# RDLLab/posggym-baselines

Measured on AMD Instinct MI355X. Metric: MCTS simulations/sec on Driving-v1 (POMCP exact search), higher is better.
Workload: dtype f64

## Files before the change

### posggym-baselines_amd/csrc/driving.h

```cpp
#pragma once
#include <stdint.h>

#include "philox.h"

namespace pb {

enum : int { NORTH = 0, EAST = 1, SOUTH = 2, WEST = 3 };
enum : int { REVERSE = 0, STOPPED = 1, FORWARD_SLOW = 2, FORWARD_FAST = 3 };
enum : int { DO_NOTHING = 0, ACCELERATE = 1, DECELERATE = 2, TURN_RIGHT = 3, TURN_LEFT = 4 };
enum : int { CELL_VEHICLE = 0, CELL_WALL = 1, CELL_EMPTY = 2, CELL_DEST = 3 };

struct DrvGrid {
  uint8_t wall[256];
  uint8_t dist[8][256];
  uint8_t loc_x[8], loc_y[8], loc_dir[8];
  int32_t width, height, num_locs;
  int32_t obs_front, obs_back, obs_side;
  int32_t pad[2];
};

struct Veh {
  int x, y, dir, speed, dest, reached, crashed, mind, initd;
};

// ... 140 lines not shown
  v.crashed = 0;
  v.mind = g.dist[dest][(v.y << 4) | v.x];
  v.initd = v.mind;
  return pack_veh(v);
}

PB_HD int kth_bit(uint32_t mask, uint32_t k) {
  for (int i = 0; i < 8; ++i) {
    if (mask & (1u << i)) {
      if (k == 0) return i;
      --k;
    }
  }
  return -1;
}

PB_HD int popc8(uint32_t m) {
  int n = 0;
  for (int i = 0; i < 8; ++i) n += (m >> i) & 1;
  return n;
}

template <class G, class Draw>
PB_HD void drv_sample_initial_state2(const G& g, Draw draw, uint32_t* s0, uint32_t* s1) {
  const uint32_t all = (1u << g.num_locs) - 1u;
  uint32_t starts = 0, dests = 0;
  uint32_t out[2];
  for (int i = 0; i < 2; ++i) {
    const uint32_t av = all & ~starts;
    const int s = kth_bit(av, draw((uint32_t)popc8(av)));
    starts |= 1u << s;
    const uint32_t avd = all & ~dests & ~(1u << s);
    const int d = kth_bit(avd, draw((uint32_t)popc8(avd)));
    dests |= 1u << d;
    out[i] = make_vehicle(g, s, d);
  }
  *s0 = out[0];
  *s1 = out[1];
}

template <class G>
PB_HD int loc_index(const G& g, int x, int y) {
  for (int k = 0; k < g.num_locs; ++k)
    if (g.loc_x[k] == x && g.loc_y[k] == y) return k;
  return -1;
}

}

namespace pb {

struct DrvModel {
  DrvGrid g;
  uint16_t win_wall[1024];
  uint16_t nbr2[1024];
  double prog[3 * 128];
};

template <class G>
PB_HD void build_model_tables(const G& g, DrvModel* m) {
  const int ncells = (g.obs_front + g.obs_back + 1) * (2 * g.obs_side + 1);
  for (int cell = 0; cell < 256; ++cell) {
    const int x = cell & 15, y = cell >> 4;
    for (int d = 0; d < 4; ++d) {
      const int nx = x + dir_dx(d), ny = y + dir_dy(d);
      int n1 = 0xFF, n2 = 0xFF;
      if (grid_free(g, nx, ny)) {
        n1 = (ny << 4) | nx;
        const int mx = nx + dir_dx(d), my = ny + dir_dy(d);
        if (grid_free(g, mx, my)) n2 = (my << 4) | mx;
      }
      m->nbr2[cell * 4 + d] = (uint16_t)(n1 | (n2 << 8));
      uint32_t w = 0;
      const int W = 2 * g.obs_side + 1;
      const int r = (d + 1) & 3;
      for (int c = 0; c < ncells; ++c) {
        const int fwd = g.obs_front - c / W;
        const int side = c % W - g.obs_side;
        const int cx = x + fwd * dir_dx(d) + side * dir_dx(r);
        const int cy = y + fwd * dir_dy(d) + side * dir_dy(r);
        if (!grid_free(g, cx, cy)) w |= 1u << c;
      }
      m->win_wall[cell * 4 + d] = (uint16_t)w;
    }
  }
  for (int k = 0; k < 3; ++k)
    for (int i = 0; i < 128; ++i)
      m->prog[k * 128 + i] = i == 0 ? 0.0 : (0.5 * (double)k) / (double)i;
}

PB_HD int window_index(const DrvGrid& g, int x, int y, int d, int tx, int ty) {
  const int rx = tx - x, ry = ty - y;
  const int r = (d + 1) & 3;
  const int fwd = rx * dir_dx(d) + ry * dir_dy(d);
  const int side = rx * dir_dx(r) + ry * dir_dy(r);
  if (fwd < -g.obs_back || fwd > g.obs_front || side < -g.obs_side || side > g.obs_side) return -1;
  return (g.obs_front - fwd) * (2 * g.obs_side + 1) + (side + g.obs_side);
}

PB_HD uint32_t spread_bits16(uint32_t x) {
  x &= 0xFFFFu;
  x = (x | (x << 8)) & 0x00FF00FFu;
  x = (x | (x << 4)) & 0x0F0F0F0Fu;
  x = (x | (x << 2)) & 0x33333333u;
  x = (x | (x << 1)) & 0x55555555u;
  return x;
}

PB_HD uint64_t obs_key_fast(const DrvModel& m, uint32_t self, uint32_t other) {
  const DrvGrid& g = m.g;
  const int ncells = (g.obs_front + g.obs_back + 1) * (2 * g.obs_side + 1);
  const uint32_t full = (1u << ncells) - 1u;
  const int x = self & 15, y = (self >> 4) & 15, d = (self >> 8) & 3;
  const uint32_t wall = m.win_wall[(((y << 4) | x) << 2) | d];
  uint32_t cells = spread_bits16(wall) | (spread_bits16(~wall & full) << 1);
  const int dest = (self >> 12) & 7;
  const int cd = window_index(g, x, y, d, g.loc_x[dest], g.loc_y[dest]);
  if (cd >= 0 && !((wall >> cd) & 1u)) cells |= 3u << (2 * cd);
  const int cv = window_index(g, x, y, d, (int)(other & 15), (int)((other >> 4) & 15));
  if (cv >= 0 && !((wall >> cv) & 1u)) cells &= ~(3u << (2 * cv));
  return (uint64_t)cells | obs_tail(g, self);
}

struct MovePlan {
  uint32_t self;
  int d, speed, cells;
  uint32_t path;
  bool done;
};

PB_HD MovePlan plan_move(const DrvModel& m, uint32_t self, int action) {
  MovePlan p;
  p.self = self;
  p.done = veh_done(self);
  int d = (self >> 8) & 3, speed = (self >> 10) & 3;
  if (action == TURN_RIGHT) d = (d + 1) & 3;
  else if (action == TURN_LEFT) d = (d + 3) & 3;
  else if (action == ACCELERATE) speed = speed + 1 < FORWARD_FAST ? speed + 1 : FORWARD_FAST;
  else if (action == DECELERATE) speed = speed - 1 > REVERSE ? speed - 1 : REVERSE;
  const int move = speed != REVERSE ? d : ((d + 2) & 3);
  p.d = d;
  p.speed = speed;
  p.cells = speed > STOPPED ? speed - STOPPED : STOPPED - speed;
  p.path = m.nbr2[((self & 0xFF) << 2) | (uint32_t)move];
  return p;
}

PB_HD int resolve_move(const MovePlan& p, int ocell, int* speed, bool* hit) {
  int cell = (int)(p.self & 0xFF);
  *speed = p.speed;
  *hit = false;
  if (p.cells >= 1) {
    const int c1 = (int)(p.path & 0xFF);
    if (c1 == 0xFF) {
      *speed = STOPPED;
    } else if (c1 == ocell) {
      *hit = true;
      *speed = STOPPED;
    } else {
      cell = c1;
      if (p.cells >= 2) {
        const int c2 = (int)(p.path >> 8);
        if (c2 == 0xFF) {
          *speed = STOPPED;
        } else if (c2 == ocell) {
          *hit = true;
          *speed = STOPPED;
        } else {
          cell = c2;
        }
      }
    }
  }
  return cell;
}

PB_HD uint32_t finish_move(const DrvModel& m, const MovePlan& p, int cell, int speed, bool hit) {
  const uint32_t self = p.self;
  const int dest = (self >> 12) & 7;
  const int dist = m.g.dist[dest][cell];
  const int mind0 = (self >> 17) & 127;
  const int mind = mind0 < dist ? mind0 : dist;
  return (self & 0x7F007000u) | (uint32_t)cell | ((uint32_t)p.d << 8) | ((uint32_t)speed << 10) |
         ((uint32_t)(dist == 0) << 15) | ((uint32_t)hit << 16) | ((uint32_t)mind << 17);
}

PB_HD void drv_step2_fast(const DrvModel& m, uint32_t s0, uint32_t s1, int a0, int a1, uint32_t j,
                          uint32_t* o0, uint32_t* o1) {
  const MovePlan p0 = plan_move(m, s0, a0);
  const MovePlan p1 = plan_move(m, s1, a1);
  const bool first1 = j == 0;
  const MovePlan& pf = first1 ? p1 : p0;
  const MovePlan& ps = first1 ? p0 : p1;
  uint32_t vf = pf.self, vs = ps.self;
  int cf = (int)(vf & 0xFF), cs = (int)(vs & 0xFF);
  int spf = 0, sps = 0;
  bool hf = false, hs = false, sec_crashed = false, fst_crashed = false;
  bool movedf = false, moveds = false;
  if (!pf.done) {
    cf = resolve_move(pf, cs, &spf, &hf);
    movedf = true;
    if (hf && !ps.done) sec_crashed = true;
  }
  if (!ps.done && !sec_crashed) {
    cs = resolve_move(ps, cf, &sps, &hs);
    moveds = true;
    if (hs) fst_crashed = true;
  }
  if (movedf) vf = finish_move(m, pf, cf, spf, hf);
  if (moveds) vs = finish_move(m, ps, cs, sps, hs);
  if (sec_crashed) vs |= 1u << 16;
  if (fst_crashed && !veh_done(vf)) vf |= 1u << 16;
  *o0 = first1 ? vs : vf;
  *o1 = first1 ? vf : vs;
}

PB_HD double drv_reward_fast(const DrvModel& m, uint32_t prev, uint32_t next) {
  if (veh_done(prev)) return 0.0;
  const double base = ((next >> 16) & 1) ? -1.0 : (((next >> 15) & 1) ? 0.5 : 0.0);
  const int progress = (int)((prev >> 17) & 127) - (int)((next >> 17) & 127);
  return base + m.prog[progress * 128 + (int)((prev >> 24) & 127)];
}

}
```

### posggym-baselines_amd/csrc/driving_vec.h

```cpp
#pragma once
#if defined(__HIPCC__)
#include <hip/hip_runtime.h>
#endif
#include <stdint.h>

#include "driving.h"

namespace pb {

PB_HD uint32_t vary(uint32_t x) {
#if defined(__HIP_DEVICE_COMPILE__)
  uint32_t r;
  asm("v_mov_b32 %0, %1" : "=v"(r) : "v"(x));
  return r;
#else
  return x;
#endif
}

struct VPlan {
  uint32_t self, path;
  uint32_t d, speed, cells, done;
};

// ... 21 lines not shown
struct VMove {
  uint32_t cell, speed, hit;
};

PB_HD VMove vresolve(const VPlan& p, uint32_t ocell) {
  const uint32_t c1 = p.path & 0xFFu, c2 = p.path >> 8;
  const uint32_t start = p.self & 0xFFu;
  const bool s1 = p.cells >= 1u;
  const bool w1 = c1 == 0xFFu, h1 = !w1 & (c1 == ocell);
  const bool a1 = s1 & !w1 & !h1;
  const bool s2 = (p.cells >= 2u) & a1;
  const bool w2 = c2 == 0xFFu, h2 = !w2 & (c2 == ocell);
  const bool a2 = s2 & !w2 & !h2;
  VMove r;
  r.cell = a2 ? c2 : (a1 ? c1 : start);
  r.hit = ((s1 & h1) | (s2 & h2)) ? 1u : 0u;
  r.speed = ((s1 & (w1 | h1)) | (s2 & (w2 | h2))) ? (uint32_t)STOPPED : p.speed;
  return r;
}

PB_HD uint32_t vfinish(const VPlan& p, const VMove& mv, uint32_t dist) {
  const uint32_t mind0 = (p.self >> 17) & 127u;
  const uint32_t mind = mind0 < dist ? mind0 : dist;
  return (p.self & 0x7F007000u) | mv.cell | (p.d << 8) | (mv.speed << 10) |
         ((dist == 0u ? 1u : 0u) << 15) | (mv.hit << 16) | (mind << 17);
}

PB_HD void drv_step2_vec(const DrvModel& m, uint32_t s0, uint32_t s1, uint32_t a0, uint32_t a1,
                         uint32_t j, uint32_t* o0, uint32_t* o1) {
  const bool first1 = j == 0u;
  const VPlan pf = vplan(m, first1 ? s1 : s0, first1 ? a1 : a0);
  const VPlan ps = vplan(m, first1 ? s0 : s1, first1 ? a0 : a1);
  const VMove mf = vresolve(pf, ps.self & 0xFFu);
  const bool movef = pf.done == 0u;
  const bool sec_crash = movef & (mf.hit != 0u) & (ps.done == 0u);
  const uint32_t cellf = movef ? mf.cell : (pf.self & 0xFFu);
  const VMove ms = vresolve(ps, cellf);
  const bool moves = (ps.done == 0u) & !sec_crash;
  const uint32_t cells = moves ? ms.cell : (ps.self & 0xFFu);
  const uint32_t distf = m.g.dist[(pf.self >> 12) & 7u][cellf];
  const uint32_t dists = m.g.dist[(ps.self >> 12) & 7u][cells];
  const uint32_t kf = movef ? ~0u : 0u, ks = moves ? ~0u : 0u;
  uint32_t vf = (vfinish(pf, mf, distf) & kf) | (pf.self & ~kf);
  uint32_t vs = (vfinish(ps, ms, dists) & ks) | (ps.self & ~ks);
  vs |= sec_crash ? (1u << 16) : 0u;
  const bool fst_crash = moves & (ms.hit != 0u) & (((vf >> 15) & 3u) == 0u);
  vf |= fst_crash ? (1u << 16) : 0u;
  *o0 = first1 ? vs : vf;
  *o1 = first1 ? vf : vs;
}

PB_HD double drv_reward_vec(const DrvModel& m, uint32_t prev, uint32_t next) {
  const uint32_t initd = (prev >> 24) & 127u;
  const double p1 = m.prog[128u + initd], p2 = m.prog[256u + initd];
  const bool done0 = ((prev >> 15) & 3u) != 0u;
  const double base = ((next >> 16) & 1u) ? -1.0 : (((next >> 15) & 1u) ? 0.5 : 0.0);
  const uint32_t progress = ((prev >> 17) & 127u) - ((next >> 17) & 127u);
  const double r = base + (progress == 1u ? p1 : (progress == 2u ? p2 : 0.0));
  return done0 ? 0.0 : r;
}

PB_HD int vwindow_index(const DrvGrid& g, int x, int y, int fx, int fy, int rx,
                                             int ry, int tx, int ty) {
  const int dx = tx - x, dy = ty - y;
  const int fwd = dx * fx + dy * fy;
  const int side = dx * rx + dy * ry;
  const bool in = fwd >= -g.obs_back && fwd <= g.obs_front && side >= -g.obs_side &&
                  side <= g.obs_side;
  return in ? (g.obs_front - fwd) * (2 * g.obs_side + 1) + (side + g.obs_side) : -1;
}

PB_HD uint64_t obs_key_vec(const DrvModel& m, uint32_t self, uint32_t other) {
  const DrvGrid& g = m.g;
  const int ncells = (g.obs_front + g.obs_back + 1) * (2 * g.obs_side + 1);
  const uint32_t full = (1u << ncells) - 1u;
  const int x = (int)(self & 15u), y = (int)((self >> 4) & 15u), d = (int)((self >> 8) & 3u);
  const uint32_t wall = m.win_wall[(self & 0xFFu) << 2 | (uint32_t)d];
  uint32_t cells = spread_bits16(wall) | (spread_bits16(~wall & full) << 1);
  const int fx = d == EAST ? 1 : (d == WEST ? -1 : 0);
  const int fy = d == SOUTH ? 1 : (d == NORTH ? -1 : 0);
  const int rx = -fy, ry = fx;
  const uint32_t dest = (self >> 12) & 7u;
  const int dxl = g.loc_x[dest], dyl = g.loc_y[dest];
  const int cd = vwindow_index(g, x, y, fx, fy, rx, ry, dxl, dyl);
  const uint32_t dmask = (cd >= 0 && !((wall >> (cd & 31)) & 1u)) ? (3u << (2 * (cd & 15))) : 0u;
  cells |= dmask;
  const int cv = vwindow_index(g, x, y, fx, fy, rx, ry, (int)(other & 15u), (int)((other >> 4) & 15u));
  const uint32_t vmask = (cv >= 0 && !((wall >> (cv & 31)) & 1u)) ? (3u << (2 * (cv & 15))) : 0u;
  cells &= ~vmask;
  const uint64_t tail = ((uint64_t)((self >> 10) & 3u) << 30) | ((uint64_t)x << 32) |
                        ((uint64_t)y << 36) | ((uint64_t)dxl << 40) | ((uint64_t)dyl << 44) |
                        ((uint64_t)((self >> 15) & 1u) << 48) | ((uint64_t)((self >> 16) & 1u) << 49);
  return (uint64_t)cells | tail;
}

}
```

### posggym-baselines_amd/csrc/pomcp_search.hip

```cpp
#pragma clang fp contract(off)

namespace pb {

constexpr int kMaxA = 5;
constexpr int kTPB = 256;
constexpr int kTPBSmall = 64;
#ifndef POMCP_ROOT_SLOTS_LDS
#define POMCP_ROOT_SLOTS_LDS 1
#endif
#ifndef POMCP_WAVES_PER_EU
#define POMCP_WAVES_PER_EU 1
#endif
constexpr bool kRootSlotsInLds = POMCP_ROOT_SLOTS_LDS != 0;
constexpr int kRootParts = kMaxA * (kRootSlotsInLds ? 1 + kSlots : 1);
__host__ __device__ constexpr int rc_stats(int a) { return a; }
__host__ __device__ constexpr int rc_slot(int a, int k) { return kMaxA + a * kSlots + k; }

constexpr int kRegPath = 3;
#ifndef PB_BQ_LEVELS
#define PB_BQ_LEVELS 3
#endif
constexpr int kBq = PB_BQ_LEVELS;
static_assert(kBq >= 1 && kBq <= kRegPath, "only register-path levels are queued (level() passes ql = -1 below)");
constexpr int kPre = 2 + kMaxA;
// ... 48 lines not shown
#endif
  const int wave = bx * (TPB / kWave) + (int)(threadIdx.x >> 6);
  const int tree = wave * kWave + lane;
  const bool valid = tree < p.B;
  const int tt = valid ? tree : 0;
  constexpr int A = NA;
  constexpr int L = blk_lines(NA, TM);
  char* const an = reinterpret_cast<char*>(p.an + tree_base_lines(tt, p.Nb, L));
  const int64_t blk_bytes = blk_stride_lines(L) * 128;
  const WaveLog wl(p.plog, p.Np, wave, TM);
  __shared__ __attribute__((aligned(16))) char tm_lds[TM != 0 ? sizeof(TmTables) : 16];
  if constexpr (TM != 0) {
    const uint32_t* src = reinterpret_cast<const uint32_t*>(p.tmt);
    uint32_t* dst = reinterpret_cast<uint32_t*>(tm_lds);
    for (int i = (int)threadIdx.x; i < (int)(sizeof(TmTables) / 4); i += TPB) dst[i] = src[i];
    __syncthreads();
  }
  const TmTables* const tmt = reinterpret_cast<const TmTables*>(tm_lds);
  uint32_t pid = 0;
  int epol = 0;
  const int islots = p.islots;
  const uint32_t slot_mask = (1u << islots) - 1u;
  const uint32_t wpos0 = p.wlog[wave];
  bool app = false;
  LogRec rec = {0u, 0u, 0u};
  __shared__ uint32_t wcnt[TPB / kWave];
  if (lane == 0) wcnt[threadIdx.x >> 6] = wpos0;
  __builtin_amdgcn_wave_barrier();
  auto append = [&]() {
    if (app) {
#ifndef POMCP_ABLATE_LOG
      const uint32_t at = atomicAdd(&wcnt[threadIdx.x >> 6], 1u);
      wl.store(at, rec);
      if constexpr (TM != 0) wl.aux[at] = pid;
#endif
      app = false;
    }
  };
  OvfSlot* const ovf = p.ovf + (int64_t)tt * p.H;
  PathEntry* const path = reinterpret_cast<PathEntry*>(p.path) + (int64_t)tt * kMaxPath;
  const TreeHdr* const h = p.hdr + tt;
  const int bdir = h->belief_sel ? -1 : 1;
  const uint4* const rbel = p.belief + (int64_t)tt * p.Nr + (h->belief_sel ? p.Nr - 1 : 0);
  int root_blk = h->root_blk, root_visits = h->root_visits;
  int n_blocks = h->n_blocks, n_log = h->n_log, n_nodes = h->n_nodes;
  const int bsize = h->belief_size, epoch = h->epoch, root_abs = h->root_abs;
  int err = h->error;
  double mm_min = h->mm_min, mm_max = h->mm_max;
  const uint64_t seed = uni64(h->seed);
  const uint32_t tkey = h->tree_key;
  uint32_t c_bel = h->ctr[0], c_sel = h->ctr[1], c_mod = h->ctr[2], c_a0 = h->ctr[3],
           c_a1 = h->ctr[4];
  const int log0 = n_log, blocks0 = n_blocks, nodes0 = n_nodes;
  int c_rollout = 0, c_probes = 0, c_cut = 0, c_exact = 0;
#ifdef POMCP_PHASE_TIMING
  uint64_t pt[16];
  for (int i = 0; i < 16; ++i) pt[i] = 0;
  uint64_t pt_last = __builtin_amdgcn_s_memtime();
#endif

  auto d_belief = [&](uint32_t n) { return uniform_int(philox_word(seed, tkey, S_BELIEF, c_bel++), n); };
  auto d_select = [&](uint32_t n) { return uniform_int(philox_word(seed, tkey, S_SELECT, c_sel++), n); };
  auto d_act_word = [&](int agent) {
    const bool a0 = agent == 0;
    const uint32_t j = a0 ? c_a0 : c_a1;
    c_a0 += a0 ? 1u : 0u;
    c_a1 += a0 ? 0u : 1u;
    return philox_word(seed, tkey, (uint32_t)S_ACT_BASE + (a0 ? 0u : 1u), j);
  };
  __shared__ uint32_t rw[2][4][TPB];
  uint32_t m_base = 0u, o_base = 0u;
  uint32_t w_bel = 0u;
  int pend_b = 0;
  uint32_t nm0 = 0u, nm1 = 0u, nm2 = 0u, nm3 = 0u, no0 = 0u, no1 = 0u, no2 = 0u, no3 = 0u;
  uint32_t nm_base = 0xFFFFFFFFu, no_base = 0xFFFFFFFFu;
  auto spec_blocks = [&]() {
    const uint32_t cm = m_base + 4u, co = o_base + 4u;
    uint32_t bo[4] = {co >> 2, 0u, (uint32_t)(S_ACT_BASE + p.other), (uint32_t)(seed >> 32)};
    philox4x32(bo, (uint32_t)seed, tkey);
    no0 = bo[0];
    no1 = bo[1];
    no2 = bo[2];
    no3 = bo[3];
    no_base = co;
    if constexpr (Env::kStepDraws) {
      uint32_t bm[4] = {cm >> 2, 0u, (uint32_t)S_MODEL, (uint32_t)(seed >> 32)};
      philox4x32(bm, (uint32_t)seed, tkey);
      nm0 = bm[0];
      nm1 = bm[1];
      nm2 = bm[2];
      nm3 = bm[3];
      nm_base = cm;
    }
  };
  auto sim_blocks = [&]() {
    c_mod = (c_mod + 3u) & ~3u;
    c_a0 = (c_a0 + 3u) & ~3u;
    c_a1 = (c_a1 + 3u) & ~3u;
    const uint32_t co = p.other == 0 ? c_a0 : c_a1;
    const bool hit = co == no_base && (!Env::kStepDraws || c_mod == nm_base);
    if (!hit) {
      uint32_t bo[4] = {co >> 2, 0u, (uint32_t)(S_ACT_BASE + p.other), (uint32_t)(seed >> 32)};
      philox4x32(bo, (uint32_t)seed, tkey);
      no0 = bo[0];
      no1 = bo[1];
      no2 = bo[2];
// ... 5 lines not shown
        nm1 = bm[1];
        nm2 = bm[2];
        nm3 = bm[3];
      }
    }
    o_base = co;
    m_base = c_mod;
    rw[0][0][lid] = nm0;
    rw[0][1][lid] = nm1;
    rw[0][2][lid] = nm2;
    rw[0][3][lid] = nm3;
    rw[1][0][lid] = no0;
    rw[1][1][lid] = no1;
    rw[1][2][lid] = no2;
    rw[1][3][lid] = no3;
  };
  static_assert(kRegPath + 1 <= 4, "DL <= kRegPath: the steps of a simulation fit one Philox block");
  auto blk_word = [&](int q, uint32_t k, uint32_t sid, uint32_t j) -> uint32_t {
    uint32_t x = rw[q][k & 3u][lid];
    if constexpr (DL == 0) {
      if (k >= 4u) x = philox_word(seed, tkey, sid, j);
    }
    return x;
  };
  auto la_bel = [&]() {
    if (!pend_b) {
      w_bel = philox_word(seed, tkey, S_BELIEF, c_bel++);
      pend_b = 1;
    }
  };
  auto take_oth = [&]() -> uint32_t {
    const bool o0 = p.other == 0;
    const uint32_t j = o0 ? c_a0 : c_a1;
    const uint32_t w = blk_word(1, j - o_base, (uint32_t)S_ACT_BASE + (o0 ? 0u : 1u), j);
    c_a0 += o0 ? 1u : 0u;
    c_a1 += o0 ? 0u : 1u;
    if constexpr (TM != 0) {
      if (tmt->other_uniform) return uniform_int(w, (uint32_t)A);
      return (uint32_t)tm_choice(tmt->oth_cum[pid], tmt->oth_tot[pid], A, w);
    } else {
      return uniform_int(w, (uint32_t)A);
    }
  };
  auto take_mod = [&](uint32_t n) -> uint32_t {
    if constexpr (Env::kStepDraws) {
      const uint32_t w = blk_word(0, c_mod - m_base, (uint32_t)S_MODEL, c_mod);
      ++c_mod;
      return uniform_int(w, n);
    } else {
      return 0u;
    }
  };
  auto alloc_block = [&](int code) -> int {
    if (n_blocks >= p.Nb) {
      err = POMCP_E_ARENA;
      return -1;
    }
    const int b = n_blocks++;
    uint4* d = reinterpret_cast<uint4*>(an + (int64_t)b * blk_bytes);
    for (int q = 0; q < blk_parts(A + 1); ++q) d[q] = make_uint4(0, 0, 0, 0);
    if constexpr (TM != 0) {
      double* const pr = reinterpret_cast<double*>(d + part_prior(A));
      for (int q = 0; q < A; ++q) pr[q] = tmt->prior[code][q];
    }
    return b;
  };

  auto select_action = [&](const uint4 (&st)[kMaxA], int nv, double log_n,
                           const double (&ap)[kMaxA]) -> int {
    int a = 0;
    if (SEL == POMCP_SEL_PUCB && nv == 0) {
      double cum[kMaxA], acc = 0.0;
#pragma unroll
      for (int q = 0; q < kMaxA; ++q) {
        const double w = TM != 0 ? ap[q] : 1.0 / (double)A;
        acc = q == 0 ? w : acc + w;
        cum[q] = acc;
      }
      const double x = uniform_float(philox_word(seed, tkey, S_SELECT, c_sel++)) * (cum[A - 1] + 0.0);
      a = A - 1;
      for (int q = 0; q < A - 1; ++q) {
        if (x < cum[q]) {
          a = q;
          break;
        }
      }
    } else if (nv == 0) {
      a = (int)d_select((uint32_t)A);
    } else if (SEL == POMCP_SEL_UNIFORM) {
      int min_n = nv + 1;
#pragma unroll
      for (int q = 0; q < A; ++q) {
        if ((int)st[q].x < min_n) {
          min_n = (int)st[q].x;
          a = q;
        }
      }
    } else {
      const bool nz = mm_max > mm_min;
      const double range = mm_max - mm_min;
      double sc[A];
      bool exact = true;
      if (SEL == POMCP_SEL_UCB) {
        if (nv >= p.logtab_n) err = POMCP_E_ARENA;
#ifdef POMCP_ABLATE_SELECT
#pragma unroll
        for (int q = 0; q < A; ++q)
          sc[q] = hilo_d(st[q].z, st[q].w) + p.c * log_n * (double)(int)st[q].x;
#else
        {
          const double rr = nz ? rcp_nr(range) : 1.0;
          const double csl = p.c * sqrt_fast(log_n);
          double sf[A], mg[A];
#pragma unroll
          for (int q = 0; q < A; ++q) {
            const double v = hilo_d(st[q].z, st[q].w);
            const int n = (int)st[q].x > 0 ? (int)st[q].x : 1;
            const double qf = nz ? (v - mm_min) * rr : v;
            const double ef = csl * rsq_nr((double)n);
            sf[q] = qf + ef;
            mg[q] = __builtin_fabs(qf) + ef;
          }
          int af = 0;
          double bf = sf[0], bm = mg[0];
          uint4 sb = st[0];
#pragma unroll
          for (int q = 1; q < A; ++q) {
            if (sf[q] > bf) {
              bf = sf[q];
              bm = mg[q];
              af = q;
            }
          }
#pragma unroll
          for (int q = 1; q < A; ++q) sb = sel4(q == af, st[q], sb);
          bool amb = false;
#pragma unroll
          for (int q = 0; q < A; ++q) {
            const bool same = st[q].x == sb.x && st[q].z == sb.z && st[q].w == sb.w;
            amb |= q != af && !same && !(bf - sf[q] > p.sel_margin * (mg[q] + bm));
          }
          a = af;
          exact = amb;
#ifdef POMCP_EXACT_SELECT
          exact = true;
#endif
        }
        if (exact) {
#pragma unroll
          for (int q = 0; q < A; ++q) {
            const double v = hilo_d(st[q].z, st[q].w);
            const double nvq = nz ? (v - mm_min) / range : v;
            const int n = (int)st[q].x > 0 ? (int)st[q].x : 1;
            sc[q] = nvq + p.c * sqrt(log_n / (double)n);
          }
        }
#endif
      } else {
        const double noise = 1.0 / (double)A;
        const double sqrt_n = sqrt((double)nv);
        double cp[A];
#pragma unroll
        for (int q = 0; q < A; ++q)
          cp[q] = p.c * ((TM != 0 ? ap[q] : 1.0 / (double)A) * (1.0 - p.pucb_f) + p.pucb_f * noise);
#ifndef POMCP_EXACT_SELECT
        {
          const double rr = nz ? rcp_nr(range) : 1.0;
          double sf[A], mg[A];
#pragma unroll
          for (int q = 0; q < A; ++q) {
            const int n = (int)st[q].x;
            const double v = hilo_d(st[q].z, st[q].w);
            const double qf = n > 0 ? (nz ? (v - mm_min) * rr : v) : 0.0;
            const double ef = cp[q] * (sqrt_n * rcp_nr((double)(1 + n)));
            sf[q] = qf + ef;
            mg[q] = __builtin_fabs(qf) + __builtin_fabs(ef);
          }
          int af = 0;
          double bf = sf[0], bm = mg[0], bp = cp[0];
          uint4 sb = st[0];
#pragma unroll
          for (int q = 1; q < A; ++q) {
            if (sf[q] > bf) {
              bf = sf[q];
              bm = mg[q];
              af = q;
            }
          }
#pragma unroll
          for (int q = 1; q < A; ++q) {
            sb = sel4(q == af, st[q], sb);
            bp = q == af ? cp[q] : bp;
          }
          bool amb = false;
#pragma unroll
          for (int q = 0; q < A; ++q) {
            const bool same = st[q].x == sb.x && st[q].z == sb.z && st[q].w == sb.w && cp[q] == bp;
            amb |= q != af && !same && !(bf - sf[q] > p.sel_margin * (mg[q] + bm));
          }
          a = af;
          exact = amb;
        }
#endif
        if (exact) {
#pragma unroll
          for (int q = 0; q < A; ++q) {
            const int n = (int)st[q].x;
            const double v = hilo_d(st[q].z, st[q].w);
            const double nvq = nz ? (v - mm_min) / range : v;
            sc[q] = (n > 0 ? nvq : 0.0) + cp[q] * (sqrt_n / (double)(1 + n));
          }
        }
      }
      if (exact) {
        ++c_exact;
        a = 0;
        double best = sc[0];
#pragma unroll
        for (int q = 1; q < A; ++q) {
          if (sc[q] > best) {
            best = sc[q];
            a = q;
          }
        }
      }
      if (SEL == POMCP_SEL_UCB) {
        int unv = -1;
#pragma unroll
        for (int q = A - 1; q >= 0; --q)
          if (st[q].x == 0u) unv = q;
        if (unv >= 0) a = unv;
      }
    }
    return a;
  };

  int phase = TP_START, sims = 0, max_depth = 0;
  int t = 0, depth = 0, plen = 0, blk = 0, nvis = 0, k = 0, rdepth = 0;
  uint32_t s0 = 0, s1 = 0;
  int32_t* leaf_ptr = nullptr;
  int leaf_rc = -1;
  double ret = 0.0;
  uint4 pf = make_uint4(0, 0, 0, 0);
  int r0_on = 0;
  uint32_t r0_a = 0, r0_vis = 0;
  double r0_r = 0.0, r0_val = 0.0, r0_tot = 0.0;
  double rt[kMaxA];
#pragma unroll
  for (int q = 0; q < kMaxA; ++q) rt[q] = 0.0;
  double rap[kMaxA];
#pragma unroll
// ... 171 lines not shown
      if (b < 0) {
        phase = TP_DONE;
      } else {
        if (leaf_rc >= 0) rc[leaf_rc][lid].z = (uint32_t)b;
        else *leaf_ptr = b;
        lf_b = b;
        lf_nv = (uint32_t)cvis;
        lf_ln = logtab(cvis + 1);
        ret = 0.0;
        k = 0;
        rdepth = depth;
        phase = TP_ROLL;
      }
    } else {
      phase = TP_LEVEL;
      const uint4* const cp = reinterpret_cast<const uint4*>(an + (int64_t)blk * blk_bytes);
#pragma unroll
      for (int q = 0; q < kPre; ++q) pre[q] = q < 2 + A ? cp[q] : make_uint4(0, 0, 0, 0);
      if constexpr (TM != 0) {
#pragma unroll
        for (int q = 0; q < 3; ++q) ppr[q] = cp[part_prior(A) + q];
      }
    }
  };
  auto prior_ema = [&](double (&ap)[kMaxA], int nv) {
#pragma unroll
    for (int q = 0; q < kMaxA; ++q)
      if (q < A) ap[q] = ap[q] + (tmt->prior[epol + 1][q] - ap[q]) / (double)nv;
  };
  auto bump_node = [&](int cb) {
    q_flush();
    uint4* const c1 = reinterpret_cast<uint4*>(an + (int64_t)cb * blk_bytes) + 1;
    const uint4 x = *c1;
    const double ln = logtab((int)x.y + 2);
    *c1 = make_uint4(x.x, x.y + 1u, (uint32_t)__double2loint(ln), (uint32_t)__double2hiint(ln));
  };
  auto push_path = [&](auto dc, PathEntry pe) {
    constexpr int D = decltype(dc)::value;
    if constexpr (D > 0) {
      rpath[D - 1] = pe;
      plen = D;
    } else {
      if (plen < kRegPath) {
#pragma unroll
        for (int l = 0; l < kRegPath; ++l)
          if (plen == l) rpath[l] = pe;
      } else {
        path[plen] = pe;
      }
      ++plen;
    }
  };

  for (int it = 0; it < num_sims; ++it) {
    PT_MARK(7);
    if (phase == TP_START) {
      {
        const uint4 pr = pf;
        if (sims + 1 < num_sims) {
#ifdef POMCP_ABLATE_BELIEF
          pf.w += uniform_int(w_bel, (uint32_t)bsize) & 1u;
#else
          pf = rbel[bdir * (int)uniform_int(w_bel, (uint32_t)bsize)];
#endif
          pend_b = 0;
        }
        t = (int)pr.x;
        s0 = pr.y;
        s1 = pr.z;
        depth = 0;
        plen = 0;
        r0_on = 0;
        sim_blocks();
        if constexpr (TM != 0) {
          pid = pr.w;
          if (!tmt->no_meta_draw) {
            const int i = tm_choice(tmt->meta_cum[pid], tmt->meta_tot[pid], tmt->meta_len[pid],
                                    philox_word(seed, tkey, S_SELECT, c_sel++));
            epol = tmt->meta_idx[pid][i];
          }
        }
        if (0 > p.depth_limit || t > p.step_limit) {
          ret = 0.0;
          phase = TP_BACKUP;
        } else {
          const uint32_t j = take_mod(2);
          const uint32_t ao = take_oth();
          uint4 st[kMaxA];
#pragma unroll
          for (int q = 0; q < kMaxA; ++q) st[q] = q < A ? rc[rc_stats(q)][lid] : make_uint4(0, 0, 0, 0);
          const int a = select_action(st, root_visits, root_logn, rap);
          uint4 sa = st[0];
          uint4 sl[kSlots];
#pragma unroll
          for (int q = 1; q < kMaxA; ++q)
            sa = sel4(q == a, st[q], sa);
#pragma unroll
          for (int q = 0; q < kSlots; ++q)
            sl[q] = kRootSlotsInLds ? rc[rc_slot(a, q)][lid] : rb[part_slot(a, q)];
          r0_tot = rt[0];
#pragma unroll
          for (int q = 1; q < kMaxA; ++q) r0_tot = q == a ? rt[q] : r0_tot;
          uint32_t n0, n1;
          double r;
          int done;
          uint64_t okey;
#ifdef POMCP_ABLATE_ROOTSTEP
          n0 = s0;
          n1 = s1;
          r = 0.0;
          done = 0;
          okey = (uint64_t)ao;
#else
          tree_step(a, ao, j, &n0, &n1, &r, &done, &okey, true);
#endif
          bool match;
          const int ks = find_slot(sl, okey, &match);
          const uint32_t ani = (uint32_t)(root_blk * A + a);
          uint32_t cid = 0;
          int cblk = -1, cvis = 1, ccode = epol + 1, existed = 0;
          if (ks >= 0) {
            uint4 sk = sl[0];
#pragma unroll
            for (int q = 1; q < kSlots; ++q)
              sk = sel4(q == ks, sl[q], sk);
            cblk = match ? (int)sk.z : cblk;
            cvis = match ? (int)sk.w + 1 : cvis;
            n_nodes += match ? 0 : 1;
            existed = match ? 1 : 0;
            if (match && cblk >= 0 && done) bump_node(cblk);
            uint64_t nk = okey | kValidBit | ((uint64_t)done << 63);
            if constexpr (TM != 0) {
              ccode = match ? (int)((sk.y >> (kCodeShift - 32)) & 15u) : ccode;
              nk |= (uint64_t)ccode << kCodeShift;
            }
            const uint4 nsl = make_uint4((uint32_t)nk, (uint32_t)(nk >> 32), (uint32_t)cblk, (uint32_t)cvis);
            cid = ani * kSlots + (uint32_t)ks + 1u;
            if (kRootSlotsInLds) {
              rc[rc_slot(a, ks)][lid] = nsl;
              leaf_rc = rc_slot(a, ks);
            } else {
              uint4* slot = const_cast<uint4*>(rb) + part_slot(a, ks);
              *slot = nsl;
              leaf_ptr = reinterpret_cast<int32_t*>(slot) + 2;
              leaf_rc = -1;
            }
          } else {
            const OvfChild o = ovf_child(ani, okey, done, cblk, cvis, ccode);
            cid = o.cid;
            cblk = o.cblk;
            cvis = o.cvis;
            ccode = o.code;
            existed = o.existed;
            leaf_ptr = o.cptr;
            leaf_rc = -1;
            if (cblk >= 0 && done) bump_node(cblk);
          }
          if constexpr (TM != 0) {
            if (existed) prior_ema(rap, root_visits);
          }
          if (err != 0 || n_log >= p.Np) {
            if (err == 0) err = POMCP_E_ARENA;
            phase = TP_DONE;
          } else {
            rec = LogRec{cid | ((uint32_t)lane << kIdBits), n0, n1};
            app = true;
            ++n_log;
            r0_on = 1;
            r0_a = (uint32_t)a | ((uint32_t)done << 31);
            r0_vis = sa.x;
            r0_r = r;
            r0_val = hilo_d(sa.z, sa.w);
            descend(DepthC<(DL > 0 ? 1 : 0)>{}, done, cblk, cvis, n0, n1, ccode);
          }
        }
      }
      root_logn = logtab(root_visits + 1);
      fw_on = q_n > 0 && phase == TP_LEVEL;
      if constexpr (DL == 0) {
        fw_b = q_b[0];
        fw_a = q_a[0];
        fw_v = q_v[0];
        fw_s1 = q_s1[0];
        fw_vt = q_vt[0];
      }
      q_flush();
      PT_MARK(0);
    }
    if (phase != TP_DONE) {
      la_bel();
      spec_blocks();
    }
    auto level_pass = [&](auto dc) __attribute__((always_inline)) {
      constexpr int D = decltype(dc)::value;
      static_assert(D >= 1 && D <= DL, "unrolled passes: depths 1..DL");
#include "pomcp_search_level.inc"
    };
    if constexpr (DL == 0) {
      while (__ballot(phase == TP_LEVEL) != 0ull) {
        constexpr int D = 0;
        DepthC<0> dc;
#include "pomcp_search_level.inc"
      }
    } else {
      if (__ballot(phase == TP_LEVEL) != 0ull) level_pass(DepthC<1>{});
      if constexpr (DL >= 2) {
        if (__ballot(phase == TP_LEVEL) != 0ull) level_pass(DepthC<2>{});
      }
      if constexpr (DL >= 3) {
        if (__ballot(phase == TP_LEVEL) != 0ull) level_pass(DepthC<3>{});
      }
      static_assert(kRegPath == 3, "one unrolled pass per register-path level");
    }
    append();
    while (phase == TP_ROLL) {
      if (!(rdepth <= p.depth_limit && t <= p.step_limit)) {
        phase = TP_BACKUP;
      } else {
        const uint32_t aw = d_act_word(p.ego);
        uint32_t ae;
        if constexpr (TM != 0)
          ae = tmt->ego_uniform ? uniform_int(aw, (uint32_t)A)
                                : (uint32_t)tm_choice(tmt->ego_cum[epol], tmt->ego_tot[epol], A, aw);
        else ae = uniform_int(aw, (uint32_t)A);
        const uint32_t j = take_mod(2);
        const uint32_t ao = take_oth();
        uint32_t n0, n1;
        double r;
        int dn;
        Env::step(sm, p.ego, s0, s1, ae, ao, j, &n0, &n1, &r, &dn);
        if (k >= p.dpow_n) {
          err = POMCP_E_ARENA;
          phase = TP_DONE;
        } else {
          ret += p.dpow[k] * r;
          ++c_rollout;
          if (dn) {
            phase = TP_BACKUP;
          } else {
            s0 = n0;
            s1 = n1;
            ++t;
            ++rdepth;
            ++k;
          }
        }
      }
      PT_MARK(5);
    }
    if (phase == TP_BACKUP) {
      double gr = ret;
      auto level = [&](auto qc, const PathEntry& pe, int ql) {
        constexpr int QC = decltype(qc)::value;
        const uint4 e0 = pe.e0, e1 = pe.e1, e2 = pe.e2;
        const double r = hilo_d(e0.z, e0.w);
        gr = (e0.x >> 31) ? r : r + p.discount * gr;
        const int n = (int)e0.y + 1;
        const double value0 = hilo_d(e1.x, e1.y);
        const double total = hilo_d(e1.z, e1.w) + gr;
        const double delta = gr - value0;
        const double value = value0 + delta / (double)n;
        const uint32_t ba = e0.x & 0x7FFFFFFFu;
        const uint32_t a = ba & 7u;
        const uint4 s1w = make_uint4(a == 4u ? (uint32_t)n : e2.x, e2.y, e2.z, e2.w);
        const uint4 vtw = make_uint4((uint32_t)__double2loint(value), (uint32_t)__double2hiint(value),
                                     (uint32_t)__double2loint(total), (uint32_t)__double2hiint(total));
        if constexpr (DL > 0 && QC < NQ) {
          q_b[QC] = (int)(ba >> 3);
          q_a[QC] = a;
          q_v[QC] = (uint32_t)n;
          q_s1[QC] = s1w;
          q_vt[QC] = vtw;
        } else {
          if (DL > 0 || ql < 0 || ql >= kBq) {
            char* const lp = an + (int64_t)(ba >> 3) * blk_bytes;
            if (a < 4u) reinterpret_cast<uint32_t*>(lp)[a] = (uint32_t)n;
            reinterpret_cast<uint4*>(lp)[1] = s1w;
            reinterpret_cast<uint4*>(lp)[part_vt((int)a)] = vtw;
          } else {
#pragma unroll
            for (int l = 0; l < kBq; ++l) {
              if (l == ql) {
                q_b[l] = (int)(ba >> 3);
                q_a[l] = a;
                q_v[l] = (uint32_t)n;
                q_s1[l] = s1w;
                q_vt[l] = vtw;
              }
            }
          }
        }
        if (value > mm_max) mm_max = value;
        if (value < mm_min) mm_min = value;
      };
      if constexpr (DL > 0) {
        if constexpr (DL >= 3) {
          if (2 < plen) level(DepthC<2>{}, rpath[2], 2);
        }
        if constexpr (DL >= 2) {
          if (1 < plen) level(DepthC<1>{}, rpath[1], 1);
        }
        if (0 < plen) level(DepthC<0>{}, rpath[0], 0);
      } else {
        for (int l = plen - 1; l >= kRegPath; --l) level(DepthC<-1>{}, path[l], -1);
        q_flush();
#pragma unroll
        for (int l = kRegPath - 1; l >= 0; --l)
          if (l < plen) level(DepthC<-1>{}, rpath[l], l);
      }
      q_n = plen < NQ ? plen : NQ;
      if (lf_b >= 0) {
        reinterpret_cast<uint4*>(an + (int64_t)lf_b * blk_bytes)[1] =
            make_uint4(0u, lf_nv, (uint32_t)__double2loint(lf_ln), (uint32_t)__double2hiint(lf_ln));
        lf_b = -1;
      }
      if (r0_on) {
        const int a = (int)(r0_a & 0x7FFFFFFFu);
        gr = (r0_a >> 31) ? r0_r : r0_r + p.discount * gr;
        const int n = (int)r0_vis + 1;
        const double total = r0_tot + gr;
        const double delta = gr - r0_val;
        const double value = r0_val + delta / (double)n;
        rc[rc_stats(a)][lid] = make_uint4((uint32_t)n, 0u, (uint32_t)__double2loint(value),
                                          (uint32_t)__double2hiint(value));
#pragma unroll
        for (int q = 0; q < kMaxA; ++q) rt[q] = q == a ? total : rt[q];
        if (value > mm_max) mm_max = value;
        if (value < mm_min) mm_min = value;
      }
      ++root_visits;
      max_depth = depth > max_depth ? depth : max_depth;
      ++sims;
      phase = TP_START;
      PT_MARK(6);
    }
  }
#ifdef POMCP_PHASE_TIMING
  if (p.timing != nullptr && (threadIdx.x & (kWave - 1)) == 0 && wave * kWave < p.B) {
    for (int i = 0; i < 16; ++i) p.timing[wave * 16 + i] = pt[i];
  }
#endif

  q_flush();
  {
    uint32_t mine = valid ? (uint32_t)(n_log - log0) : 0u;
#pragma unroll
    for (int o = 32; o >= 1; o >>= 1) mine += (uint32_t)__shfl_xor((int)mine, o);
    if (lane == 0) p.wlog[wave] = wpos0 + mine;
  }
  if (!valid) return;
  if (cached) {
    uint4* const wb = const_cast<uint4*>(rb);
    uint32_t vw[kMaxA];
#pragma unroll
    for (int a = 0; a < kMaxA; ++a) {
      vw[a] = 0u;
      if (a < A) {
        const uint4 s = rc[rc_stats(a)][lid];
        vw[a] = s.x;
        wb[part_vt(a)] = make_uint4(s.z, s.w, (uint32_t)__double2loint(rt[a]), (uint32_t)__double2hiint(rt[a]));
        if (kRootSlotsInLds) {
#pragma unroll
          for (int q = 0; q < kSlots; ++q) wb[part_slot(a, q)] = rc[rc_slot(a, q)][lid];
        }
      }
    }
    wb[0] = make_uint4(vw[0], vw[1], vw[2], vw[3]);
    reinterpret_cast<uint32_t*>(wb)[4] = vw[4];
    if constexpr (TM != 0) {
#pragma unroll
      for (int a = 0; a < kMaxA; ++a)
        if (a < A) reinterpret_cast<double*>(wb + part_prior(A))[a] = rap[a];
    }
  }
  const bool have = err == 0 && !root_abs && root_blk >= 0;
  uint4 st[kMaxA];
  double tot[kMaxA];
  {
    const uint4* const hb = reinterpret_cast<const uint4*>(an + (int64_t)(have ? root_blk : 0) * blk_bytes);
    uint4 p0 = make_uint4(0, 0, 0, 0), p1 = p0;
    if (have && !cached) {
      p0 = hb[0];
      p1 = hb[1];
    }
#pragma unroll
    for (int a = 0; a < kMaxA; ++a) {
      st[a] = make_uint4(0, 0, 0, 0);
      tot[a] = 0.0;
      if (have && a < A) {
        if (cached) {
          st[a] = rc[rc_stats(a)][lid];
          tot[a] = rt[a];
        } else {
          const uint4 vt = hb[part_vt(a)];
          st[a] = make_uint4(line_visits(p0, p1, a), 0u, vt.x, vt.y);
          tot[a] = hilo_d(vt.z, vt.w);
// ... 178 lines not shown
```

### posggym-baselines_amd/csrc/pomcp_search_level.inc

```
      if (phase == TP_LEVEL) {
        const uint4* const ap = reinterpret_cast<const uint4*>(an + (int64_t)blk * blk_bytes);
        const uint32_t j = take_mod(2);
        const uint32_t ao = take_oth();
        PT_MARK(8);
        if constexpr (D <= 1) {
          if (fw_on) {
            fw_on = false;
            if (blk == (D == 1 ? q_b[0] : fw_b)) {
              const uint32_t a4 = D == 1 ? q_a[0] : fw_a, v4 = D == 1 ? q_v[0] : fw_v;
              pre[0] = make_uint4(a4 == 0u ? v4 : pre[0].x, a4 == 1u ? v4 : pre[0].y,
                                  a4 == 2u ? v4 : pre[0].z, a4 == 3u ? v4 : pre[0].w);
              pre[1] = D == 1 ? q_s1[0] : fw_s1;
#pragma unroll
              for (int q = 2; q < kPre; ++q)
                pre[q] = sel4(q == part_vt((int)a4), D == 1 ? q_vt[0] : fw_vt, pre[q]);
            }
          }
        }
        nvis = (int)pre[1].y + 1;
        const double log_n = hilo_d(pre[1].z, pre[1].w);
        const double lnx = logtab(nvis + 1);
        uint4 st[kMaxA];
  #pragma unroll
        for (int q = 0; q < kMaxA; ++q)
// ... 32 lines not shown
        uint64_t okey;
        tree_step(a, ao, j, &n0, &n1, &r, &done, &okey, !skipc);
        bool match = false;
        int ks = 0;
        if ((D > 0 && D < DL) || !skipc) ks = find_slot(sl, okey, &match);
        PT_MARK(12);
        const uint32_t ani = (uint32_t)(blk * A + a);
        uint32_t cid = 0;
        int cblk = -1, cvis = 1, ccode = epol + 1, existed = 0;
        leaf_rc = -1;
        if (skipc) {
          cid = p.cut_base + ani;
        } else if (ks >= 0) {
          uint4 sk = sl[0];
  #pragma unroll
          for (int q = 1; q < kSlots; ++q)
            sk = sel4(q == ks, sl[q], sk);
          cblk = match ? (int)sk.z : cblk;
          cvis = match ? (int)sk.w + 1 : cvis;
          n_nodes += match ? 0 : 1;
          existed = match ? 1 : 0;
          uint64_t nk = okey | kValidBit | ((uint64_t)done << 63);
          if constexpr (TM != 0) {
            ccode = match ? (int)((sk.y >> (kCodeShift - 32)) & 15u) : ccode;
            nk |= (uint64_t)ccode << kCodeShift;
          }
          uint4* slot = const_cast<uint4*>(ap) + part_slot(a, ks);
          const bool flip = (sk.y >> 31) != (uint32_t)done;
          if (!match || flip || (cblk < 0 && (done || !cutc)))
            *slot = make_uint4((uint32_t)nk, (uint32_t)(nk >> 32), (uint32_t)cblk, (uint32_t)cvis);
          if (match && cblk >= 0 && done) bump_node(cblk);
          cid = ani * kSlots + (uint32_t)ks + 1u;
          leaf_ptr = reinterpret_cast<int32_t*>(slot) + 2;
        } else {
          const OvfChild o = ovf_child(ani, okey, done, cblk, cvis, ccode);
          cid = o.cid;
          cblk = o.cblk;
          cvis = o.cvis;
          ccode = o.code;
          existed = o.existed;
          leaf_ptr = o.cptr;
          if (cblk >= 0 && done) bump_node(cblk);
        }
        if constexpr (TM != 0) {
          if (existed) {
            prior_ema(lap, nvis);
            double* const pl = reinterpret_cast<double*>(const_cast<uint4*>(ap) + part_prior(A));
#pragma unroll
            for (int q = 0; q < kMaxA; ++q)
              if (q < A) pl[q] = lap[q];
          }
        }
        PT_MARK(13);
        if (err != 0 || n_log >= p.Np || (D > 0 ? false : plen >= kMaxPath)) {
          if (err == 0) err = POMCP_E_ARENA;
          phase = TP_DONE;
        } else {
          rec = LogRec{cid | ((uint32_t)lane << kIdBits), n0, n1};
          app = true;
          ++n_log;
          const uint32_t ba = ((uint32_t)blk << 3) | (uint32_t)a;
          push_path(dc, PathEntry{
              make_uint4(ba | ((uint32_t)done << 31), sa.x, (uint32_t)__double2loint(r),
                         (uint32_t)__double2hiint(r)),
              va,
              make_uint4(pre[1].x, (uint32_t)nvis, (uint32_t)__double2loint(lnx),
                         (uint32_t)__double2hiint(lnx))});
          PT_MARK(14);
          descend(DepthC<(D > 0 ? D + 1 : 0)>{}, done, cblk, cvis, n0, n1, ccode);
        }
        PT_MARK(4);
      }
```

Before: 7.214 billion.

## Precompute spread window table, simplify obs key, and hoist search params into registers

Stores the pre-spread 2-bit-per-cell wall window in the model table so the obs key no longer spreads bits at runtime. The window index is rebuilt from a branchless heading decomposition that uses packed geometry and destination tables. The progress-reward table is collapsed to a single row, with the half-weight case derived by multiplication. The search loop now holds UCB constants, the block cap and a countdown of log room in VGPRs, which is meant to avoid repeated scalar loads and 64-bit compares. The cost is a larger window table and somewhat more register pressure.

```diff
diff --git a/posggym-baselines_amd/csrc/driving.h b/posggym-baselines_amd/csrc/driving.h
--- a/posggym-baselines_amd/csrc/driving.h
+++ b/posggym-baselines_amd/csrc/driving.h
@@ -216,10 +216,22 @@
 
 struct DrvModel {
   DrvGrid g;
-  uint16_t win_wall[1024];
+  uint32_t win2[1024];
   uint16_t nbr2[1024];
-  double prog[3 * 128];
+  double prog[128];
+  uint8_t loc_xy[8];
+  alignas(16) int32_t win_geo[4];
 };
+static_assert(sizeof(DrvModel) == sizeof(DrvGrid) + 4096 + 2048 + 1024 + 8 + 16, "no padding");
+
+PB_HD uint32_t spread_bits16(uint32_t x) {
+  x &= 0xFFFFu;
+  x = (x | (x << 8)) & 0x00FF00FFu;
+  x = (x | (x << 4)) & 0x0F0F0F0Fu;
+  x = (x | (x << 2)) & 0x33333333u;
+  x = (x | (x << 1)) & 0x55555555u;
+  return x;
+}
 
 template <class G>
 PB_HD void build_model_tables(const G& g, DrvModel* m) {
@@ -245,12 +257,16 @@
         const int cy = y + fwd * dir_dy(d) + side * dir_dy(r);
         if (!grid_free(g, cx, cy)) w |= 1u << c;
       }
-      m->win_wall[cell * 4 + d] = (uint16_t)w;
-    }
-  }
-  for (int k = 0; k < 3; ++k)
-    for (int i = 0; i < 128; ++i)
-      m->prog[k * 128 + i] = i == 0 ? 0.0 : (0.5 * (double)k) / (double)i;
+      const uint32_t full = (1u << ncells) - 1u;
+      m->win2[cell * 4 + d] = spread_bits16(w) | (spread_bits16(~w & full) << 1);
+    }
+  }
+  for (int k = 0; k < 8; ++k) m->loc_xy[k] = (uint8_t)((g.loc_x[k] & 15) | ((g.loc_y[k] & 15) << 4));
+  m->win_geo[0] = g.obs_front;
+  m->win_geo[1] = g.obs_front + g.obs_back + 1;
+  m->win_geo[2] = g.obs_side;
+  m->win_geo[3] = 2 * g.obs_side + 1;
+  for (int i = 0; i < 128; ++i) m->prog[i] = i == 0 ? 0.0 : (0.5 * 2.0) / (double)i;
 }
 
 PB_HD int window_index(const DrvGrid& g, int x, int y, int d, int tx, int ty) {
@@ -262,27 +278,15 @@
   return (g.obs_front - fwd) * (2 * g.obs_side + 1) + (side + g.obs_side);
 }
 
-PB_HD uint32_t spread_bits16(uint32_t x) {
-  x &= 0xFFFFu;
-  x = (x | (x << 8)) & 0x00FF00FFu;
-  x = (x | (x << 4)) & 0x0F0F0F0Fu;
-  x = (x | (x << 2)) & 0x33333333u;
-  x = (x | (x << 1)) & 0x55555555u;
-  return x;
-}
-
 PB_HD uint64_t obs_key_fast(const DrvModel& m, uint32_t self, uint32_t other) {
   const DrvGrid& g = m.g;
-  const int ncells = (g.obs_front + g.obs_back + 1) * (2 * g.obs_side + 1);
-  const uint32_t full = (1u << ncells) - 1u;
   const int x = self & 15, y = (self >> 4) & 15, d = (self >> 8) & 3;
-  const uint32_t wall = m.win_wall[(((y << 4) | x) << 2) | d];
-  uint32_t cells = spread_bits16(wall) | (spread_bits16(~wall & full) << 1);
+  uint32_t cells = m.win2[(((y << 4) | x) << 2) | d];
   const int dest = (self >> 12) & 7;
   const int cd = window_index(g, x, y, d, g.loc_x[dest], g.loc_y[dest]);
-  if (cd >= 0 && !((wall >> cd) & 1u)) cells |= 3u << (2 * cd);
+  if (cd >= 0 && ((cells >> (2 * cd + 1)) & 1u)) cells |= 3u << (2 * cd);
   const int cv = window_index(g, x, y, d, (int)(other & 15), (int)((other >> 4) & 15));
-  if (cv >= 0 && !((wall >> cv) & 1u)) cells &= ~(3u << (2 * cv));
+  if (cv >= 0 && ((cells >> (2 * cv + 1)) & 1u)) cells &= ~(3u << (2 * cv));
   return (uint64_t)cells | obs_tail(g, self);
 }
 
@@ -383,7 +387,8 @@
   if (veh_done(prev)) return 0.0;
   const double base = ((next >> 16) & 1) ? -1.0 : (((next >> 15) & 1) ? 0.5 : 0.0);
   const int progress = (int)((prev >> 17) & 127) - (int)((next >> 17) & 127);
-  return base + m.prog[progress * 128 + (int)((prev >> 24) & 127)];
-}
-
-}
+  const double p2 = m.prog[(prev >> 24) & 127];
+  return base + (progress == 1 ? 0.5 * p2 : (progress == 2 ? p2 : 0.0));
+}
+
+}
diff --git a/posggym-baselines_amd/csrc/driving_vec.h b/posggym-baselines_amd/csrc/driving_vec.h
--- a/posggym-baselines_amd/csrc/driving_vec.h
+++ b/posggym-baselines_amd/csrc/driving_vec.h
@@ -97,7 +97,7 @@
 
 PB_HD double drv_reward_vec(const DrvModel& m, uint32_t prev, uint32_t next) {
   const uint32_t initd = (prev >> 24) & 127u;
-  const double p1 = m.prog[128u + initd], p2 = m.prog[256u + initd];
+  const double p2 = m.prog[initd], p1 = 0.5 * p2;
   const bool done0 = ((prev >> 15) & 3u) != 0u;
   const double base = ((next >> 16) & 1u) ? -1.0 : (((next >> 15) & 1u) ? 0.5 : 0.0);
   const uint32_t progress = ((prev >> 17) & 127u) - ((next >> 17) & 127u);
@@ -105,38 +105,32 @@
   return done0 ? 0.0 : r;
 }
 
-PB_HD int vwindow_index(const DrvGrid& g, int x, int y, int fx, int fy, int rx,
-                                             int ry, int tx, int ty) {
-  const int dx = tx - x, dy = ty - y;
-  const int fwd = dx * fx + dy * fy;
-  const int side = dx * rx + dy * ry;
-  const bool in = fwd >= -g.obs_back && fwd <= g.obs_front && side >= -g.obs_side &&
-                  side <= g.obs_side;
-  return in ? (g.obs_front - fwd) * (2 * g.obs_side + 1) + (side + g.obs_side) : -1;
+static_assert(NORTH == 0 && EAST == 1 && SOUTH == 2 && WEST == 3, "heading order");
+
+PB_HD uint32_t vwindow_bits(const int32_t (&geo)[4], uint32_t cells, bool horiz, int kf, int ks,
+                            int dx, int dy) {
+  const int along = horiz ? dx : dy, across = horiz ? dy : dx;
+  const uint32_t row = (uint32_t)(geo[0] - ((along ^ kf) - kf));
+  const uint32_t col = (uint32_t)(((across ^ ks) - ks) + geo[2]);
+  const uint32_t sh = (2u * (row * (uint32_t)geo[3] + col)) & 31u;
+  const bool in = (row < (uint32_t)geo[1]) & (col < (uint32_t)geo[3]);
+  const uint32_t k = (in & ((((cells >> sh) >> 1) & 1u) != 0u)) ? ~0u : 0u;
+  return (3u << sh) & k;
 }
 
 PB_HD uint64_t obs_key_vec(const DrvModel& m, uint32_t self, uint32_t other) {
-  const DrvGrid& g = m.g;
-  const int ncells = (g.obs_front + g.obs_back + 1) * (2 * g.obs_side + 1);
-  const uint32_t full = (1u << ncells) - 1u;
-  const int x = (int)(self & 15u), y = (int)((self >> 4) & 15u), d = (int)((self >> 8) & 3u);
-  const uint32_t wall = m.win_wall[(self & 0xFFu) << 2 | (uint32_t)d];
-  uint32_t cells = spread_bits16(wall) | (spread_bits16(~wall & full) << 1);
-  const int fx = d == EAST ? 1 : (d == WEST ? -1 : 0);
-  const int fy = d == SOUTH ? 1 : (d == NORTH ? -1 : 0);
-  const int rx = -fy, ry = fx;
-  const uint32_t dest = (self >> 12) & 7u;
-  const int dxl = g.loc_x[dest], dyl = g.loc_y[dest];
-  const int cd = vwindow_index(g, x, y, fx, fy, rx, ry, dxl, dyl);
-  const uint32_t dmask = (cd >= 0 && !((wall >> (cd & 31)) & 1u)) ? (3u << (2 * (cd & 15))) : 0u;
-  cells |= dmask;
-  const int cv = vwindow_index(g, x, y, fx, fy, rx, ry, (int)(other & 15u), (int)((other >> 4) & 15u));
-  const uint32_t vmask = (cv >= 0 && !((wall >> (cv & 31)) & 1u)) ? (3u << (2 * (cv & 15))) : 0u;
-  cells &= ~vmask;
-  const uint64_t tail = ((uint64_t)((self >> 10) & 3u) << 30) | ((uint64_t)x << 32) |
-                        ((uint64_t)y << 36) | ((uint64_t)dxl << 40) | ((uint64_t)dyl << 44) |
-                        ((uint64_t)((self >> 15) & 1u) << 48) | ((uint64_t)((self >> 16) & 1u) << 49);
-  return (uint64_t)cells | tail;
+  const uint32_t d = (self >> 8) & 3u;
+  uint32_t cells = m.win2[(self & 0xFFu) << 2 | d];
+  const uint32_t dxy = m.loc_xy[(self >> 12) & 7u];
+  const int32_t geo[4] = {m.win_geo[0], m.win_geo[1], m.win_geo[2], m.win_geo[3]};
+  const int x = (int)(self & 15u), y = (int)((self >> 4) & 15u);
+  const bool horiz = (d & 1u) != 0u;
+  const int kf = (int)(((d + 1u) >> 1) & 1u) - 1;
+  const int ks = -(int)(d >> 1);
+  cells |= vwindow_bits(geo, cells, horiz, kf, ks, (int)(dxy & 15u) - x, (int)(dxy >> 4) - y);
+  cells &= ~vwindow_bits(geo, cells, horiz, kf, ks, (int)(other & 15u) - x, (int)((other >> 4) & 15u) - y);
+  const uint32_t hi = (self & 0xFFu) | (dxy << 8) | (((self >> 15) & 3u) << 16);
+  return (uint64_t)(cells | (((self >> 10) & 3u) << 30)) | ((uint64_t)hi << 32);
 }
 
 }
diff --git a/posggym-baselines_amd/csrc/pomcp_search.hip b/posggym-baselines_amd/csrc/pomcp_search.hip
--- a/posggym-baselines_amd/csrc/pomcp_search.hip
+++ b/posggym-baselines_amd/csrc/pomcp_search.hip
@@ -124,6 +124,16 @@
   uint32_t c_bel = h->ctr[0], c_sel = h->ctr[1], c_mod = h->ctr[2], c_a0 = h->ctr[3],
            c_a1 = h->ctr[4];
   const int log0 = n_log, blocks0 = n_blocks, nodes0 = n_nodes;
+  auto log_room0 = [&]() -> int {
+    const int64_t r = p.Np - (int64_t)log0;
+    return r > 0x7FFFFFFF ? 0x7FFFFFFF : (r < 0 ? 0 : (int)r);
+  };
+  int room = log_room0();
+  auto vary_d = [](double x) {
+    return __hiloint2double((int)vary((uint32_t)__double2hiint(x)), (int)vary((uint32_t)__double2loint(x)));
+  };
+  const double c_ucb = vary_d(p.c), sel_margin = vary_d(p.sel_margin), discount = vary_d(p.discount);
+  const int nb_cap = (int)vary((uint32_t)(p.Nb > 0x7FFFFFFF ? 0x7FFFFFFF : (int)p.Nb));
   int c_rollout = 0, c_probes = 0, c_cut = 0, c_exact = 0;
 #ifdef POMCP_PHASE_TIMING
   uint64_t pt[16];
@@ -235,7 +245,7 @@
     }
   };
   auto alloc_block = [&](int code) -> int {
-    if (n_blocks >= p.Nb) {
+    if (n_blocks >= nb_cap) {
       err = POMCP_E_ARENA;
       return -1;
     }
@@ -289,11 +299,11 @@
 #ifdef POMCP_ABLATE_SELECT
 #pragma unroll
         for (int q = 0; q < A; ++q)
-          sc[q] = hilo_d(st[q].z, st[q].w) + p.c * log_n * (double)(int)st[q].x;
+          sc[q] = hilo_d(st[q].z, st[q].w) + c_ucb * log_n * (double)(int)st[q].x;
 #else
         {
           const double rr = nz ? rcp_nr(range) : 1.0;
-          const double csl = p.c * sqrt_fast(log_n);
+          const double csl = c_ucb * sqrt_fast(log_n);
           double sf[A], mg[A];
 #pragma unroll
           for (int q = 0; q < A; ++q) {
@@ -321,7 +331,7 @@
 #pragma unroll
           for (int q = 0; q < A; ++q) {
             const bool same = st[q].x == sb.x && st[q].z == sb.z && st[q].w == sb.w;
-            amb |= q != af && !same && !(bf - sf[q] > p.sel_margin * (mg[q] + bm));
+            amb |= q != af && !same && !(bf - sf[q] > sel_margin * (mg[q] + bm));
           }
           a = af;
           exact = amb;
@@ -335,7 +345,7 @@
             const double v = hilo_d(st[q].z, st[q].w);
             const double nvq = nz ? (v - mm_min) / range : v;
             const int n = (int)st[q].x > 0 ? (int)st[q].x : 1;
-            sc[q] = nvq + p.c * sqrt(log_n / (double)n);
+            sc[q] = nvq + c_ucb * sqrt(log_n / (double)n);
           }
         }
 #endif
@@ -345,7 +355,7 @@
         double cp[A];
 #pragma unroll
         for (int q = 0; q < A; ++q)
-          cp[q] = p.c * ((TM != 0 ? ap[q] : 1.0 / (double)A) * (1.0 - p.pucb_f) + p.pucb_f * noise);
+          cp[q] = c_ucb * ((TM != 0 ? ap[q] : 1.0 / (double)A) * (1.0 - p.pucb_f) + p.pucb_f * noise);
 #ifndef POMCP_EXACT_SELECT
         {
           const double rr = nz ? rcp_nr(range) : 1.0;
@@ -379,7 +389,7 @@
 #pragma unroll
           for (int q = 0; q < A; ++q) {
             const bool same = st[q].x == sb.x && st[q].z == sb.z && st[q].w == sb.w && cp[q] == bp;
-            amb |= q != af && !same && !(bf - sf[q] > p.sel_margin * (mg[q] + bm));
+            amb |= q != af && !same && !(bf - sf[q] > sel_margin * (mg[q] + bm));
           }
           a = af;
           exact = amb;
@@ -657,12 +667,12 @@
     }
   };
 
-  for (int it = 0; it < num_sims; ++it) {
+  for (int left = num_sims; left > 0; --left) {
     PT_MARK(7);
     if (phase == TP_START) {
       {
         const uint4 pr = pf;
-        if (sims + 1 < num_sims) {
+        if (left > 1) {
 #ifdef POMCP_ABLATE_BELIEF
           pf.w += uniform_int(w_bel, (uint32_t)bsize) & 1u;
 #else
@@ -764,13 +774,13 @@
           if constexpr (TM != 0) {
             if (existed) prior_ema(rap, root_visits);
           }
-          if (err != 0 || n_log >= p.Np) {
+          if (err != 0 || room <= 0) {
             if (err == 0) err = POMCP_E_ARENA;
             phase = TP_DONE;
           } else {
             rec = LogRec{cid | ((uint32_t)lane << kIdBits), n0, n1};
             app = true;
-            ++n_log;
+            --room;
             r0_on = 1;
             r0_a = (uint32_t)a | ((uint32_t)done << 31);
             r0_vis = sa.x;
@@ -859,7 +869,7 @@
         constexpr int QC = decltype(qc)::value;
         const uint4 e0 = pe.e0, e1 = pe.e1, e2 = pe.e2;
         const double r = hilo_d(e0.z, e0.w);
-        gr = (e0.x >> 31) ? r : r + p.discount * gr;
+        gr = (e0.x >> 31) ? r : r + discount * gr;
         const int n = (int)e0.y + 1;
         const double value0 = hilo_d(e1.x, e1.y);
         const double total = hilo_d(e1.z, e1.w) + gr;
@@ -921,7 +931,7 @@
       }
       if (r0_on) {
         const int a = (int)(r0_a & 0x7FFFFFFFu);
-        gr = (r0_a >> 31) ? r0_r : r0_r + p.discount * gr;
+        gr = (r0_a >> 31) ? r0_r : r0_r + discount * gr;
         const int n = (int)r0_vis + 1;
         const double total = r0_tot + gr;
         const double delta = gr - r0_val;
@@ -947,6 +957,7 @@
 #endif
 
   q_flush();
+  n_log = log0 + (log_room0() - room);
   {
     uint32_t mine = valid ? (uint32_t)(n_log - log0) : 0u;
 #pragma unroll
diff --git a/posggym-baselines_amd/csrc/pomcp_search_level.inc b/posggym-baselines_amd/csrc/pomcp_search_level.inc
--- a/posggym-baselines_amd/csrc/pomcp_search_level.inc
+++ b/posggym-baselines_amd/csrc/pomcp_search_level.inc
@@ -108,13 +108,13 @@
           }
         }
         PT_MARK(13);
-        if (err != 0 || n_log >= p.Np || (D > 0 ? false : plen >= kMaxPath)) {
+        if (err != 0 || room <= 0 || (D > 0 ? false : plen >= kMaxPath)) {
           if (err == 0) err = POMCP_E_ARENA;
           phase = TP_DONE;
         } else {
           rec = LogRec{cid | ((uint32_t)lane << kIdBits), n0, n1};
           app = true;
-          ++n_log;
+          --room;
           const uint32_t ba = ((uint32_t)blk << 3) | (uint32_t)a;
           push_path(dc, PathEntry{
               make_uint4(ba | ((uint32_t)done << 31), sa.x, (uint32_t)__double2loint(r),
```

Result: no change. 7.351 billion, median of 6 (+1.9%).
